# iyak/RNAelem

Hardware: AMD Instinct MI355X
Metric: train-iter seqs/sec (inside+outside) (higher is better)
Workload: dtype f64; 1 GPU; 10000 synthetic RNAs L=200, pattern ((.*.)), W=50 C=30 min_bpp=1e-4 T2004, x0 lambda=(1,1), one (fn,gr) eval per step; n_seq=10000, seq_len=200, pattern=((.*.)), bpp_filter=cached (computed once at load_batch, 0.1 s incl. plan), n_skipped=0

## Files before the change

rnaelem_amd/csrc/lin_kernels.hip:

```cpp
#include <hip/hip_runtime.h>

#include <algorithm>
#include <cstdio>
#include <cstdlib>
#include <type_traits>

#ifndef ELEMDP_KCI
#define ELEMDP_KCI 2
#endif
#ifndef ELEMDP_LB_IN
#define ELEMDP_LB_IN 4
#endif
#ifndef ELEMDP_LB_IN_FAST
#define ELEMDP_LB_IN_FAST 8
#endif
#ifndef ELEMDP_LB_CYK
#define ELEMDP_LB_CYK 8
#endif
#ifndef ELEMDP_LB_OUT6
#define ELEMDP_LB_OUT6 6
#endif
#ifndef ELEMDP_LB_OUT
#define ELEMDP_LB_OUT 4
#endif
#ifndef ELEMDP_BAND_THREADS
#define ELEMDP_BAND_THREADS 256
#endif
#ifndef ELEMDP_CPB_MAX
#define ELEMDP_CPB_MAX 64
#endif
#ifndef ELEMDP_KIB
#define ELEMDP_KIB 4
#endif
#ifndef ELEMDP_RECIN
#define ELEMDP_RECIN 1024
#endif
#ifndef ELEMDP_RECOUT
#define ELEMDP_RECOUT 960
#endif
#include "kernels.h"
#include "lin_rules.h"
#include "lin_fast.h"
#include "lin_views.h"
#include "scan_rules.h"
#include "wave_gather.h"

namespace elemdp {
namespace {
constexpr int kBT = ELEMDP_BAND_THREADS;
constexpr int kWaves = kBT / 64;

__device__ __forceinline__ int div_small(int q, int n) { return (int)(((float)q + 0.5f) * __frcp_rn((float)n)); }
__device__ __forceinline__ int div_rcp(int q, float rcp) { return (int)(((float)q + 0.5f) * rcp); }

__device__ __forceinline__ double rep_sum(const double* p, int nrep, int stride) {
  double a = p[0];
  for (int r = 1; r < nrep; ++r) a += p[r * stride];
  return a;
}

struct LinSink {
  double* en_;
  double eh0, eh1;
  int world = 0;
  double* pos0 = nullptr;
  double* pos1 = nullptr;
  double* pos2 = nullptr;
  __device__ __forceinline__ void en(int idx, double w) { atomicAdd(&en_[idx], w); }
  __device__ __forceinline__ void eh(int k, double w) { eh1 += k ? w : 0.; eh0 += k ? 0. : w; }
  __device__ __forceinline__ void pos(int which, int p, double w) {
    double* a = (which == 0) ? pos0 : (which == 1) ? pos1 : pos2;
    if (a) atomicAdd(&a[p], w);
  }
};

struct PhaseClock {
  long long* row;
  long long t0;
  __device__ __forceinline__ void start(long long* p) {
    row = p ? p + 16 * ((blockIdx.x + 7 * blockIdx.y) & 63) : nullptr;
    t0 = 0;
    if (row) t0 = __builtin_readcyclecounter();
  }
  template <int SLOT> __device__ __forceinline__ void mark() {
    if (row) {
      const long long t = __builtin_readcyclecounter();
      if (threadIdx.x == 0) atomicAdd((unsigned long long*)&row[SLOT], (unsigned long long)(t - t0));
      t0 = t;
    }
  }
  __device__ __forceinline__ void finish() {}
};

__device__ __forceinline__ void swizzled_block(unsigned& bx, unsigned& by) {
  const unsigned nbx = gridDim.x, total = gridDim.x * gridDim.y;
  const unsigned orig = blockIdx.y * nbx + blockIdx.x;
// ... 687 lines not shown
        const int xc = x < np ? x : np - 1;
        const LoopItem it = R.it[xc];
        const int meta = R.meta[xc];
        const int c = (meta >> 16) & 0x7fff;
        const int i = ci(c), j = i + d;
        const bool in_set = x < np && meta >= 0;
        const uint32_t rP = v.in.cidx(ST_P, it.l - it.k, it.k, 0), rL1 = v.in.cidx(ST_L, it.k - i, i, 0), rL2 = v.in.cidx(ST_L, j - it.l, it.l, 0);
        const double xw0 = R.xw[xc], xw1 = R.xw[R.cap + xc];
        double* hrow = heA + c * HD;
        const int qd = FAST ? A.fqd_in : A.qd_in;
        const int m0 = a.det ? __builtin_amdgcn_readfirstlane(G[qd + wv]) : 0;
        const int n_mine = a.det ? __builtin_amdgcn_readfirstlane(G[qd + wv + 1]) - m0 : (nq > wv ? (nq - wv + kWaves - 1) / kWaves : 0);
        for (int k0 = 0; k0 < n_mine; k0 += kTU) {
          int qa[kTU], qb[kTU];
          double x0[kTU], x1[kTU], x2[kTU];
#pragma unroll
          for (int u = 0; u < kTU; ++u) {
            const bool on = k0 + u < n_mine;
            const int kk = on ? k0 + u : 0;
            const int t = a.det ? __builtin_amdgcn_readfirstlane(G[qd + 5 + m0 + kk]) : wv + kWaves * kk;
            qa[u] = __builtin_amdgcn_readfirstlane(G[qc_in + 2 * t]);
            qb[u] = on ? __builtin_amdgcn_readfirstlane(G[qc_in + 2 * t + 1]) : (4 << 16);
            x0[u] = B[rP + (qa[u] & 0xff)]; x1[u] = B[rL1 + ((qa[u] >> 8) & 0xff)]; x2[u] = B[rL2 + ((qa[u] >> 16) & 0xff)];
          }
#pragma unroll
          for (int u = 0; u < kTU; ++u) {
            const double term = x0[u] * (x1[u] * x2[u]) * ((qb[u] & (1 << 16)) ? xw1 : xw0);
            if (!(qb[u] & (4 << 16)) && in_set && term != 0.) atomicAdd(&hrow[qb[u] & 0xffff], term);
          }
        }
      }
      __syncthreads();
    }
  }
  pc.mark<3>();
  const int NL = FAST ? A.n_lane : NA;
  if (tid < nc * NL && !(a.dbg & 4) && !(ELEMDP_KO & 4)) {
    const int c = div_rcp(tid, a.rcp_lane);
    const int s = FAST ? G[A.f_live_in + tid - c * NL] : tid - c * NL;
    const int i = ci(c);
    if (FAST) {
      fast_inside_unary<kFastR, FP, kFastL, CON, LPRE>(A, G + A.fp_in + s * kFastW, v.m.lin, v.in, crec + c * kCellInD, crfl[c], d, i, hb + c * HD + (tid - c * NL),
                                                 he + c * HD + (tid - c * NL), NW, 2 * CS, G + A.fs_in);
    } else {
      const Constraint con{CON ? a.ys[v.n] : -1, -1, 0};
      lin_inside_target_u<CON>(v.m, v.q, v.in, d, i, s, rep_sum(hb + c * HD + s, NW, 2 * CS), rep_sum(he + c * HD + s, NW, 2 * CS), con);
    }
  }
  pc.mark<4>();
  pc.finish();
}

constexpr int kLoopLanes = 64;
constexpr int kLoopColsMax = 16;
constexpr int kLoopProgW = 8;
static_assert(4 + kFastR <= kLoopProgW, "the staged program holds the right transitions");
static size_t loop_prepass_lds(const AutomatonLayout& A) {
  return sizeof(double) * (2 * (size_t)kLoopLanes * A.tab_rs[ST_L] + 5 * (size_t)A.n_wr) + sizeof(int32_t) * kLoopColsMax * kLoopProgW;
}
__global__ __launch_bounds__(kLoopLanes) void k4_in_loops(LinArgs a) {
  extern __shared__ double lds[];
  LViews v(a.lay);
  make_lviews(a, blockIdx.y, v);
  const AutomatonLayout& A = a.lay;
  const int tid = threadIdx.x, L = v.q.L, W = v.q.W;
  const int i0 = blockIdx.x * kLoopLanes;
  if (i0 > L) return;
  const int rs = v.in.rs[ST_L];
  double* cur = lds;
  double* prev = lds + kLoopLanes * rs;
  double* wr = lds + 2 * kLoopLanes * rs;
  int32_t* prog = reinterpret_cast<int32_t*>(wr + 5 * A.n_wr);
  for (int t = tid; t < kLoopColsMax * kLoopProgW; t += kLoopLanes) prog[t] = 0;
  for (int t = tid; t < 5 * A.n_wr; t += kLoopLanes) wr[t] = a.lin[A.lin_wr + t];
  __syncthreads();
  for (int k = tid; k < A.n_lane; k += kLoopLanes) {
    const int32_t* P = a.ints + A.fp_in + a.ints[A.f_live_in + k] * kFastW;
    const int c = fcol(P[2], 2);
    if (c >= 0 && c < kLoopColsMax)
      for (int w = 0; w < kLoopProgW; ++w) prog[c * kLoopProgW + w] = P[w];
  }
  __syncthreads();
  const int i = i0 + tid;
  const int dmax = (W < L - i0) ? W : L - i0;
  for (int d = 0; d <= dmax; ++d) {
    if (i + d <= L) {
      const int j = i + d;
      const int bj = d > 0 ? (int)v.q.seq[j - 1] : 0;
      const double ews_j = d > 0 ? v.q.ews[j - 1] : 1.;
      const int ub = v.q.ubits(i, d);
      for (int c = 0; c < rs; ++c)
        cur[tid * rs + c] = loop_inside_entry<kFastR>(prog + c * kLoopProgW, wr, prev + tid * rs, ub, d, bj, ews_j);
    }
    __syncthreads();
    const int nrows = (kLoopLanes < L - d - i0 + 1) ? kLoopLanes : L - d - i0 + 1;
    double* dst = v.in.band + v.in.cidx(ST_L, d, i0, 0);
    for (int t = tid; t < nrows * rs; t += kLoopLanes) dst[t] = cur[t];
    double* x = cur; cur = prev; prev = x;
  }
}

struct ExtLds { int lin, ews, blob, bits, seq8, unp8, total; };
__host__ __device__ inline ExtLds ext_lds(int nd, int n_lin, int Lmax, int nword, int n_stage) {
  ExtLds b;
  int o = nd * 8;
  b.lin = o; o += n_lin * 8;
  b.ews = o; o += (Lmax + 1) * 8;
  b.blob = o; o += n_stage * 4;
// ... 832 lines not shown
            op[u] = out.lda(d + 1, i, u < nr ? ce[u] & 0xff : p, u < nr);
          }
          double acc = 0.;
          if (a_in != 0.) {
            acc = tg != 0xff ? hp[c * HD + tg] : 0.;
            const double inz = a_in * (w1 ? pi.invZs : pi.invZ);
            const int bj = step ? (int)v.q.seq[j] : 0;
            const double ewj = step ? v.q.ews[j] : 1.;
            double* en = l_en + (w1 ? nt : 0);
#pragma unroll
            for (int u = 0; u < kFastR; ++u)
              if (u < nr) {
                const int id = (ce[u] >> 8) & 0x7fff;
                const double term = op[u] * (v.m.lin[A.lin_wr + 5 * id + bj] * ((G[A.fe_r + 2 * id + 1] & 1) ? ewj : 1.));
                const double z = term * inz;
                if ((MODE == OUT_SCAN || MODE == OUT_END) &&
                    !fast_scan_stat<MODE, false, true>(sink, G[A.fs_out + id], i - 1, j, false, MODE == OUT_END && j == a.ys[v.n], L == j + 1, z))
                  continue;
                if (MODE != OUT_END && !v.m.no_prf && z != 0. && bj) atomicAdd(&en[G[A.fe_r + 2 * id] + bj], z);
                acc += term;
              }
          }
          out.a(d, i, p) = acc;
        }
        continue;
      }
      const int tgt = v.m.ints[A.ap_tgt + p];
      const bool w1 = pi.merged && v.m.ints[A.ap_t + p] == A.shadow;
      sink.en_ = l_en + (w1 ? nt : 0);
      LinOutCtx<LinSink> x{v.m, v.q, in, out, w1 ? pi.invZs : pi.invZ, sink, Constraint{MODE == OUT_END ? a.ys[v.n] : -1, -1, 0}};
      lin_outside_apair<MODE>(x, d, i0 + c, p, tgt >= 0 ? hp[c * HD + tgt] : 0.);
    }
    sink.en_ = en_keep;
  }
  pc.mark<11>();
  if (MODE == OUT_SCAN || MODE == OUT_END) {
    __syncthreads();
    const int p1 = (i0 + nc + d < L) ? i0 + nc + d : L;
    for (int t = tid; t <= p1 - pos_p0; t += kBT) {
      const double v0 = l_pos[t], v1 = l_pos[win + t];
      if (MODE == OUT_SCAN) {
        if (v0 != 0. && pos_p0 + t < L) atomicAdd(&a.pos_start[v.seq_base + pos_p0 + t], v0);
        if (v1 != 0. && pos_p0 + t < L) atomicAdd(&a.pos_inner[v.seq_base + pos_p0 + t], v1);
      } else if (v0 != 0.) {
        atomicAdd(&a.pos_end[v.pos_base + pos_p0 + t], v0);
      }
    }
  }
  if (MODE == OUT_TRAIN || MODE == OUT_SCAN) lflush(a, v, pi, sink, l_en0, kBT, (int)bx);
  pc.mark<12>();
  pc.finish();
}

constexpr int kRowsT = 8, kRowsMax = 32, kSeedCap = 256, kSeedBatch = 2;
static_assert(2 * kRowsMax <= 64, "the runs of a tile are scanned by one wave");
__host__ __device__ inline int loop_rows_r(int rs) { const int r = kBT / (rs > 0 ? rs : 1); return r < kRowsMax ? r : kRowsMax; }
static size_t loop_rows_lds(const AutomatonLayout& A) {
  const size_t rs = A.tab_rs[ST_L], R = loop_rows_r(A.tab_rs[ST_L]);
  return sizeof(double) * (R * (kRowsT + 1) * rs + 2 * kSeedCap + (R + kRowsT) + 5 * (size_t)A.n_wr + 2 * (size_t)A.n_theta + 4) +
         sizeof(int32_t) * (2 * R * (kRowsT + 1) + 2 * R + 1 + 4 * kSeedCap + 4 * (size_t)A.n_quad + (size_t)A.n_lane + kLoopColsMax * (kLoopProgW + 1) + (R + kRowsT));
}
__global__ __launch_bounds__(kBT) void k4_out_lrows(LinArgs a) {
  extern __shared__ double lds[];
  unsigned bx, by;
  swizzled_block(bx, by);
  LViews v(a.lay);
  make_lviews(a, by, v);
  const LPass pi = lpass(a, v);
  if (pi.skip) return;
  const AutomatonLayout& A = a.lay;
  const int tid = threadIdx.x, L = v.q.L, W = v.q.W, nt = A.n_theta, nq = A.n_quad, HD = A.n_lane;
  const int rs = v.out.rs[ST_L], R = loop_rows_r(rs), TS = (kRowsT + 1) * rs;
  const int i0 = bx * R;
  if (i0 > L) return;
  const int nrow = (R < L - i0 + 1) ? R : L - i0 + 1, nrr = 2 * nrow;
  double* acc = lds;
  double* s_xw = acc + R * TS;
  double* s_ew = s_xw + 2 * kSeedCap;
  double* wr = s_ew + R + kRowsT;
  double* l_en = wr + 5 * A.n_wr;
  int* offs = reinterpret_cast<int*>(l_en + 2 * nt + 4);
  int* pre = offs + 2 * R * (kRowsT + 1);
  int* s_row = pre + 2 * R + 1;
  int* tq = s_row + 4 * kSeedCap;
  int* lcol = tq + 4 * nq;
  int32_t* prog = lcol + HD;
  int32_t* pst = prog + kLoopColsMax * kLoopProgW;
  int* s_b = pst + kLoopColsMax;
  const int32_t* G = v.m.big;
  for (int t = tid; t < kLoopColsMax * (kLoopProgW + 1); t += kBT) prog[t] = 0;
  for (int t = tid; t < 5 * A.n_wr; t += kBT) wr[t] = a.lin[A.lin_wr + t];
  for (int t = tid; t < 2 * nt + 4; t += kBT) l_en[t] = 0.;
  for (int t = tid; t < 4 * nq; t += kBT) tq[t] = G[A.fqc_out + 2 * nq + t];
  __syncthreads();
  for (int k = tid; k < HD; k += kBT) {
    const int s = a.ints[A.f_live_out + k];
    const int32_t* P = a.ints + A.fp_out + s * kFastW;
    const int c = fcol(P[2], 2);
    lcol[k] = (c >= 0 && c < rs) ? c : -1;
    if (c >= 0 && c < kLoopColsMax) {
      for (int w = 0; w < kLoopProgW; ++w) prog[c * kLoopProgW + w] = P[w];
      pst[c] = s;
    }
  }
  __syncthreads();
  const int r = tid / rs, c = tid - r * rs, i = i0 + r;
  const bool lane = r < R;
  const int32_t* P = prog + (lane ? c : 0) * kLoopProgW;
  const int w0 = P[0];
  const bool have = lane && i <= L && (w0 & 1);
  const bool w1 = pi.merged && pst[lane ? c : 0] == A.shadow;
  const int kl = (w0 >> 2) & 1, cEo = fcol(P[1], 1), ehs = v.m.lam_same ? 0 : kl;
  const double invZ = w1 ? pi.invZs : pi.invZ;
  int enr[kFastR], fr[kFastR];
#pragma unroll
  for (int u = 0; u < kFastR; ++u) {
    const bool on = u < ((w0 >> 8) & 15);
    const int id = on ? (P[4 + u] >> 16) & 0x7fff : 0;
    enr[u] = on ? G[A.fe_r + 2 * id] : 0;
    fr[u] = on ? G[A.fe_r + 2 * id + 1] : 0;
  }
  LinSink sink;
  sink.world = w1 ? 1 : 0;
  sink.en_ = l_en + (w1 ? nt : 0);
  sink.eh0 = sink.eh1 = 0.;
  double* const row_e = acc + (lane ? r * TS + c : 0);
  const float rcp_nq = 1.0f / (float)(nq > 0 ? nq : 1);
  const double* IB = v.in.band;
  const double* OB = v.out.band;
  const int dmax = (W < L - i0) ? W : L - i0;
  double carry = 0.;
  for (int dhi = dmax; dhi >= 0; dhi -= kRowsT) {
    const int d0 = dhi >= kRowsT ? dhi - kRowsT + 1 : 0, nd = dhi - d0 + 1;
    double inL[kRowsT], t6[kRowsT];
    {
      int ub[kRowsT];
      uint32_t pw[kRowsT];
#pragma unroll
      for (int dd = 0; dd < kRowsT; ++dd) {
        const int d = d0 + dd;
        const bool in = have && dd < nd && i + d <= L;
        const bool up = in && i > 0 && d + 2 <= W && i + d + 1 <= L;
        ub[dd] = v.q.ubits(in ? i : 0, in ? d : 0);
        ub[dd] = in ? ub[dd] : 0;
        pw[dd] = v.q.okbits[up ? (uint32_t)v.q.cell(i - 1, d + 2) >> 5 : 0u];
        pw[dd] = up ? pw[dd] : 0u;
      }
#pragma unroll
      for (int dd = 0; dd < kRowsT; ++dd) {
        const int d = d0 + dd, c_up = v.q.cell(i - 1, d + 2);
        const bool on = (ub[dd] & UB_L) != 0, eok = on && ((pw[dd] >> (c_up & 31)) & 1u);
        inL[dd] = v.in.ldc(ST_L, d, i, c, on);
        const double oE = v.out.ldc(ST_E, d, i, cEo, eok), xhp = xw_cell(v.q, kl, XT_HP, eok ? c_up : 0), ehp = v.q.e_hp[eok ? c_up : 0];
        t6[dd] = 0.;
        if (eok && inL[dd] != 0.) t6[dd] = loop_outside_cell(inL[dd], oE, xhp, ehp, invZ, ehs, sink);
      }
    }
    if (lane) {
#pragma unroll
      for (int dd = 0; dd < kRowsT; ++dd) row_e[dd * rs] = dd == nd ? carry : t6[dd];
      row_e[kRowsT * rs] = carry;
    }
    {
      constexpr int kOffU = (2 * kRowsMax * (kRowsT + 1) + kBT - 1) / kBT;
      int ov[kOffU], os[kOffU];
#pragma unroll
      for (int u = 0; u < kOffU; ++u) {
        const int t = tid + u * kBT;
        const bool ok = t < nrr * (nd + 1) && nq > 0;
        const int rr = ok ? div_small(t, nd + 1) : 0, dd = ok ? t - rr * (nd + 1) : 0, role = rr >= nrow, d = d0 + dd;
        const int32_t* off = role ? v.q.by_right_off : v.q.by_left_off;
        os[u] = t < nrr * (nd + 1) ? rr * (kRowsT + 1) + dd : -1;
        ov[u] = off[ok ? v.q.cell(i0 + rr - role * nrow, d > 0 ? d : 1) : 0];
        ov[u] = ok ? ov[u] : 0;
      }
      int lo = 0, hi = 0;
      if (tid < 64) {
        const bool ok = tid < nrr && nq > 0;
        const int role = tid >= nrow, ri = i0 + tid - role * nrow;
        const int32_t* off = role ? v.q.by_right_off : v.q.by_left_off;
        lo = off[ok ? v.q.cell(ri, d0 > 0 ? d0 : 1) : 0];
        hi = off[ok ? v.q.cell(ri, d0 + nd) : 0];
        lo = ok ? lo : 0;
        hi = ok ? hi : 0;
      }
      int jb = 0;
      double jw = 0.;
      if (tid < nrow + nd) {
        const int j = i0 + d0 + tid;
        jb = j < L ? (int)v.q.seq[j] : 0;
        jw = v.q.ews[j < L ? j : L];
      }
#pragma unroll
      for (int u = 0; u < kOffU; ++u)
        if (os[u] >= 0) offs[os[u]] = ov[u];
      if (tid < 64) {
        int n = hi - lo;
#pragma unroll
        for (int sft = 1; sft < 64; sft <<= 1) {
          const int up = __shfl_up(n, sft);
          if (tid >= sft) n += up;
        }
        if (tid < nrr) pre[tid + 1] = n;
        if (tid == 0) pre[0] = 0;
      }
      if (tid < nrow + nd) { s_b[tid] = jb; s_ew[tid] = jw; }
    }
    __syncthreads();
    const int n_rec = pre[nrr];
    for (int p0 = 0; p0 < n_rec; p0 += kSeedCap) {
      const int np = (kSeedCap < n_rec - p0) ? kSeedCap : n_rec - p0;
      for (int xs = tid; xs < np; xs += kBT) {
        const int x = p0 + xs;
        int rr = 0;
        while (rr + 1 < nrr && pre[rr + 1] <= x) ++rr;
        const int* ro = offs + rr * (kRowsT + 1);
        const int n = ro[0] + (x - pre[rr]);
        int dd = 0;
        while (dd + 1 < nd && ro[dd + 1] <= n) ++dd;
        const int role = rr >= nrow, rw = rr - role * nrow, ri = i0 + rw, d = d0 + dd;
        const bool on = ri + d <= L && (v.q.ubits(ri, d) & UB_L);
        const LoopItem it = (role ? v.q.items_right : v.q.items_left)[n];
        s_row[xs] = (int)v.out.cidx(ST_E, it.j - it.i, it.i, 0);
        s_row[kSeedCap + xs] = (int)v.in.cidx(ST_P, it.l - it.k, it.k, 0);
        s_row[2 * kSeedCap + xs] = (int)(role ? v.in.cidx(ST_L, it.k - it.i, it.i, 0) : v.in.cidx(ST_L, it.j - it.l, it.l, 0));
        s_row[3 * kSeedCap + xs] = on ? 2 * (rw * TS + dd * rs) + role : -1;
        s_xw[xs] = lin_weight(v.m.lambda[0], it.tsc);
        s_xw[kSeedCap + xs] = lin_weight(v.m.lambda[1], it.tsc);
      }
      __syncthreads();
      for (int wb = tid; wb < np * nq; wb += kSeedBatch * kBT) {
        double x0[kSeedBatch], x1[kSeedBatch], x2[kSeedBatch], xw[kSeedBatch];
        int dst[kSeedBatch];
#pragma unroll
        for (int u = 0; u < kSeedBatch; ++u) {
          const int w = wb + u * kBT;
          const bool in = w < np * nq;
          const int xs = in ? div_rcp(w, rcp_nq) : 0, t = in ? w - xs * nq : 0;
          const int cell = s_row[3 * kSeedCap + xs];
          const int32_t* q2 = tq + (cell & 1) * 2 * nq + 2 * t;
          const int qa = q2[0], qb = q2[1], col = lcol[qb & 0xffff];
          const bool ok = in && cell >= 0 && col >= 0 && !(qb & (4 << 16));
          dst[u] = ok ? (cell >> 1) + col : -1;
          x0[u] = OB[ok ? (uint32_t)s_row[xs] + (qa & 0xff) : 0u];
          x1[u] = IB[ok ? (uint32_t)s_row[kSeedCap + xs] + ((qa >> 8) & 0xff) : 0u];
          x2[u] = IB[ok ? (uint32_t)s_row[2 * kSeedCap + xs] + ((qa >> 16) & 0xff) : 0u];
          xw[u] = s_xw[((qb >> 16) & 1) * kSeedCap + xs];
        }
#pragma unroll
        for (int u = 0; u < kSeedBatch; ++u)
          if (dst[u] >= 0) {
            const double term = loop_outside_seed_term(x0[u], x1[u], x2[u], xw[u]);
            if (term != 0.) atomicAdd(&acc[dst[u]], term);
          }
      }
      __syncthreads();
    }
    double oL = carry;
#pragma unroll
    for (int dd = kRowsT - 1; dd >= 0; --dd) {
      if (dd >= nd) continue;
      oL = 0.;
      if (inL[dd] != 0.) {
        const int d = d0 + dd, j = i + d;
        double sL = 0.;
        if (j < L && d + 1 <= W)
          sL = loop_outside_chain<kFastR>(P, enr, fr, wr, row_e + (dd + 1) * rs - c, inL[dd], s_b[r + dd], s_ew[r + dd], invZ, v.m.no_prf != 0, sink);
        oL = row_e[dd * rs] + sL;
      }
      if (lane) row_e[dd * rs] = oL;
      __syncthreads();
    }
    carry = oL;
  }
  lflush(a, v, pi, sink, l_en, kBT, (int)bx);
}

__global__ __launch_bounds__(kThreads) void k4_combine(LinArgs a, int G) {
  const int g = blockIdx.x;
  if (g >= G) return;
  const int n = a.grp[g];
  double* row = a.seq_out + (size_t)n * a.out_stride;
  if (row[4] != 0.) return;
  const double* zs = a.zs + (size_t)g * 4;
  const int nt = a.lay.n_theta;
  if (a.det) {
    const double* dr = a.det_rows + (size_t)n * a.det_nslot * a.out_stride;
    for (int t = 6 + threadIdx.x; t < 6 + 2 * nt + 4; t += kThreads) {
      double acc = 0.;
      for (int k = 0; k < a.det_nslot; ++k) acc += dr[(size_t)k * a.out_stride + t];
      row[t] = acc;
    }
    __syncthreads();
  }
  const bool positive = a.plans[n].positive != 0;
  const double pa = zs[1] / zs[0], pn = zs[2] / zs[0];
  for (int t = threadIdx.x; t < nt + 2; t += kThreads) {
    double* A = (t < nt) ? &row[6 + t] : &row[6 + 2 * nt + (t - nt)];
    double* B = (t < nt) ? &row[6 + nt + t] : &row[6 + 2 * nt + 2 + (t - nt)];
    const double va = *A, vb = *B;
    if (a.schedule == 1) {
      const double full = pa * va + pn * vb;
      if (a.lik_ratio && !positive) { *A = va; *B = full; }
      else { *A = full; *B = positive ? va : vb; }
    } else if (a.lik_ratio && !positive) {
      *A = vb; *B = va;
    }
  }
}

__device__ __forceinline__ unsigned long long cyk_key(double v) {
  const long long b = __double_as_longlong(v + 0.);
  return (unsigned long long)(b >= 0 ? b : (b ^ 0x7fffffffffffffffLL)) ^ 0x8000000000000000ULL;
}
__device__ __forceinline__ double cyk_unkey(unsigned long long k) {
  const long long b = (long long)(k ^ 0x8000000000000000ULL);
  return __longlong_as_double(b >= 0 ? b : (b ^ 0x7fffffffffffffffLL));
}

__global__ __launch_bounds__(kThreads) void k5_cyk_serial(LinArgs a) {
  __shared__ AutomatonLayout s_lay;
  stage_layout(a, &s_lay, kThreads);
  unsigned bx, by;
  swizzled_block(bx, by);
  LViews v(s_lay);
  make_lviews(a, by, v);
// ... 340 lines not shown
  switch (k4_form(a, lds, 6, fast, big)) {
    case K4_FP2_WAVES: hipLaunchKernelGGL((k4_out<MODE, true, true, 2, true>), grid, dim3(kBT), lds, st, a); break;
    case K4_FP2: hipLaunchKernelGGL((k4_out<MODE, true, true, 2>), grid, dim3(kBT), lds, st, a); break;
    case K4_FAST: hipLaunchKernelGGL((k4_out<MODE, true, true>), grid, dim3(kBT), lds, st, a); break;
    case K4_STAGED: hipLaunchKernelGGL((k4_out<MODE, true>), grid, dim3(kBT), lds, st, a); break;
    case K4_GENERIC: hipLaunchKernelGGL((k4_out<MODE, false>), grid, dim3(kBT), lds, st, a); break;
  }
}
template <>
void launch_k4_out<OUT_NONE>(const LinArgs& a, dim3 grid, size_t lds, bool, bool, hipStream_t st) {
  hipLaunchKernelGGL((k4_out<OUT_NONE, true>), grid, dim3(kBT), lds, st, a);
}

struct GroupGeom {
  LinArgs a;
  bool big, fast;
  int hd, win;
  size_t lds_in, lds_out;
  bool stage_ext;
  size_t lds_ext_in;
  int ext_nt;
};
static bool geometry_fast(const LinArgs& a) {
  return a.fast && a.n_stage >= a.lay.n_ints && a.lay.fp_ok && !(a.dbg & 16) && a.lay.lin_total <= 2048;
}
int lin_train_cpb(const LinArgs& full) {
  return geometry_fast(full) ? std::min(kBT / std::max(full.lay.n_lane, 1), ELEMDP_CPB_MAX) : 0;
}
int lin_live_span_max() { return kLiveSpanMax; }
bool lin_loop_prepass_ok(const AutomatonLayout& A, const int32_t* ints, int min_span) {
  const bool say = getenv("ELEMDP_PLAN_DEBUG") != nullptr;
  if (!A.fp_ok || A.tab_rs[ST_L] < 1 || A.tab_rs[ST_L] > kLoopColsMax || loop_prepass_lds(A) > 64 * 1024) {
    if (say) fprintf(stderr, "loop pre-pass: not for this automaton (fp_ok %d, L row of %d columns)\n", A.fp_ok, A.tab_rs[ST_L]);
    return false;
  }
  auto col = [](int packed, int byte) { const int c = (packed >> (8 * byte)) & 0xff; return c == 0xff ? -1 : c; };
  unsigned seen = 0;
  for (int k = 0; k < A.n_lane; ++k) {
    const int32_t* P = ints + A.fp_in + ints[A.f_live_in + k] * kFastW;
    const int c = col(P[2], 2);
    if (c >= 0) {
      if (c >= A.tab_rs[ST_L] || ((seen >> c) & 1u)) { if (say) fprintf(stderr, "loop pre-pass: not for this automaton (column %d of lane %d)\n", c, k); return false; }
      seen |= 1u << c;
      continue;
    }
    if (!(P[0] & 1) || col(P[1], 1) < 0) continue;
    const int nR = (P[0] >> 8) & 15;
    bool zero = !(P[0] & 2) || min_span > 2;
    for (int u = 0; u < nR && u < kFastR; ++u) zero = zero && col(P[4 + u], 0) < 0;
    if (!zero) { if (say) fprintf(stderr, "loop pre-pass: not for this automaton (lane %d: a loop state with an E column, no L column and an L value)\n", k); return false; }
  }
  return true;
}
static bool loop_outside_lds_ok(const AutomatonLayout& A) {
  return A.tab_rs[ST_L] >= 1 && A.tab_rs[ST_L] <= kLoopColsMax && A.tab_rs[ST_L] <= kBT && loop_rows_lds(A) <= 64 * 1024;
}
bool lin_loop_outside_ok(const AutomatonLayout& A, const int32_t* ints) {
  const bool say = getenv("ELEMDP_PLAN_DEBUG") != nullptr;
  if (!A.fp_ok || !loop_outside_lds_ok(A)) {
    if (say) fprintf(stderr, "L kernel behind the outside sweep: not for this automaton (fp_ok %d, L row of %d columns, LDS %zu)\n", A.fp_ok, A.tab_rs[ST_L], loop_rows_lds(A));
    return false;
  }
  auto col = [](int packed, int byte) { const int c = (packed >> (8 * byte)) & 0xff; return c == 0xff ? -1 : c; };
  unsigned seen = 0;
  for (int k = 0; k < A.n_lane; ++k) {
    const int s = ints[A.f_live_out + k];
    const int c = col(ints[A.fp_out + s * kFastW + 2], 2), ci = col(ints[A.fp_in + s * kFastW + 2], 2);
    if (c != ci || (c >= 0 && (c >= A.tab_rs[ST_L] || ((seen >> c) & 1u)))) {
      if (say) fprintf(stderr, "L kernels behind the outside sweep: not for this automaton (state %d: L column %d outside, %d inside)\n", s, c, ci);
      return false;
    }
    if (c >= 0) seen |= 1u << c;
  }
  return true;
}
static GroupGeom group_geometry(const LinArgs& full, int G, int Lmax, int Wmax, bool scan) {
  GroupGeom g;
  LinArgs& a = g.a;
  a = full;
  const int S = a.lay.S, nt = a.lay.n_theta;
  a.cpb = std::min(kBT / S, ELEMDP_CPB_MAX);
  a.wmax = Wmax;
  a.ext_ring = G <= 1024 ? 1 : 0;
  a.lmax = Lmax;
  if (scan) { a.schedule = 0; a.pass = 0; a.scan = 1; a.det = 0; }
  g.big = a.n_stage >= a.lay.n_ints;
  const bool fast = g.fast = geometry_fast(a);
  a.fast = fast ? 1 : 0;
  if (fast) a.cpb = std::min(kBT / std::max(a.lay.n_lane, 1), ELEMDP_CPB_MAX);
  a.n_lin = fast ? a.lay.lin_total : kLinEth + nt;
  const int NW = a.det ? kBT / 64 : 1;
  g.hd = fast ? a.lay.n_lane : S;
  set_rcps(a, fast);
  if (scan || !fast || a.det || !a.p.useful || !a.p.blocks || !a.blk_grid || a.live_span < a.cpb) { a.p.blocks = nullptr; a.blk_grid = nullptr; a.live_span = 0; }
  if (scan || !fast || !a.p.useful) a.loop_pre = 0;
  if (a.loop_pre && a.p.blocks && (!a.p.blocks_in || !a.blk_grid_in)) a.loop_pre = 0;
  if (scan || !fast || !a.p.useful || a.det) a.loop_post = 0;
  if (a.loop_post && a.p.blocks && (!a.p.blocks_in || !a.blk_grid_in)) a.loop_post = 0;
  if (a.loop_post && !loop_outside_lds_ok(a.lay)) a.loop_post = 0;
  const int sp = a.live_span > a.cpb ? a.live_span : a.cpb;
  g.win = sp + Wmax + 3;
  g.lds_in = block_lds(2 * a.cpb * g.hd + kRecIn, a.cpb, a.n_lin, g.win, fast ? a.lay.fb_in_n : staged_ints(a.lay, a.n_stage, 0), 0, fast ? kCellInD : 0, sp).total;
  g.lds_out = block_lds(out_doubles(a.cpb * g.hd, nt, g.win, NW, scan), a.cpb, a.n_lin, g.win, fast ? a.lay.fb_out_n : staged_ints(a.lay, a.n_stage, 1), 3 * a.cpb, fast ? kCellOutD : 0, sp).total;
  g.stage_ext = Lmax <= 2048 && a.nword_max <= 8192;
  g.lds_ext_in = g.stage_ext ? (size_t)ext_lds((a.ext_ring ? ext_ring_doubles(0, Wmax, S, kLinEth + nt, Lmax, a.nword_max, a.n_stage) : 0), kLinEth + nt, Lmax, a.nword_max, a.n_stage).total : 0;
  g.ext_nt = (a.ext_block == kExtBlock && a.ext_ring && a.lay.n_active <= 128 && !(a.dbg & 8192)) ? 128 * kExtBlock : 128;
  return g;
}
static unsigned band_blocks(LinArgs& a, int ncell, bool train) {
  const int n = (ncell + a.cpb - 1) / a.cpb;
  if (!train || !a.blk_grid || !a.p.blocks) return (unsigned)n;
  if (a.blk_grid[a.d] < 0) { a.p.blocks = nullptr; return (unsigned)n; }
  if (a.zeros_kept && a.blk_grid[a.d] == 0) return 0u;
  return (unsigned)std::max(1, std::min(n, a.blk_grid[a.d]));
}
template <bool CON>
static void inside_sweeps(GroupGeom& g, int G, int Lmax, int Wmax, bool bands, hipStream_t st) {
  LinArgs& a = g.a;
  const bool pre = !CON && bands && g.fast && a.loop_pre;
  LinArgs ai = a;
  if (!pre) ai.loop_pre = 0;
  if (pre) {
    if (a.p.blocks) { ai.p.blocks = a.p.blocks_in; ai.blk_grid = a.blk_grid_in; }
    hipLaunchKernelGGL(k4_in_loops, dim3((Lmax + kLoopLanes) / kLoopLanes, G), dim3(kLoopLanes), loop_prepass_lds(a.lay), st, ai);
  }
  if (bands)
    for (int d = pre ? a.in_d0 : 0; d <= Wmax; ++d) {
      const int ncell = Lmax - d + 1;
      if (ncell <= 0) break;
      LinArgs ad = ai;
      ad.d = d;
      const unsigned gx = band_blocks(ad, ncell, !CON);
      if (!gx) continue;
      launch_k4_in<CON>(ad, dim3(gx, G), g.lds_in, g.fast, g.big, st);
    }
  if (g.stage_ext) hipLaunchKernelGGL((k4_in_ext<true, CON>), dim3(G), dim3(g.ext_nt), g.lds_ext_in, st, a);
  else hipLaunchKernelGGL((k4_in_ext<false, CON>), dim3(G), dim3(128), 0, st, a);
}
template <int MODE>
static void outside_bands(GroupGeom& g, int G, int Lmax, int Wmax, hipStream_t st) {
  LinArgs& a = g.a;
  hipLaunchKernelGGL(k4_r7, dim3(((Lmax + 1) * (Wmax + 1) + kThreads - 1) / kThreads, G), dim3(kThreads), 0, st, a);
  const bool post = MODE == OUT_TRAIN && g.fast && a.loop_post;
  LinArgs ao = a;
  if (!post) ao.loop_post = 0;
  if (post && a.p.blocks) { ao.p.blocks = a.p.blocks_in; ao.blk_grid = a.blk_grid_in; }
  for (int d = Wmax; d >= (post ? a.in_d0 : 0); --d) {
    const int ncell = Lmax - d + 1;
    if (ncell <= 0) continue;
    LinArgs ad = ao;
    ad.d = d;
    const unsigned gx = band_blocks(ad, ncell, MODE == OUT_TRAIN);
    if (!gx) continue;
    launch_k4_out<MODE>(ad, dim3(gx, G), g.lds_out, g.fast, g.big, st);
  }
  if (post) {
    const int rows = loop_rows_r(a.lay.tab_rs[ST_L]);
    hipLaunchKernelGGL(k4_out_lrows, dim3((Lmax + rows) / rows, G), dim3(kBT), loop_rows_lds(a.lay), st, a);
  }
}
template <int MODE>
static void scan_outside(GroupGeom& g, int G, int Lmax, int Wmax, hipStream_t st) {
  const LinArgs& a = g.a;
  const int S = a.lay.S, nt = a.lay.n_theta;
  const size_t lds_ext_out = g.stage_ext ? (size_t)ext_lds(2 * nt + 4 + (a.ext_ring ? ext_ring_doubles(2 * nt + 4, Wmax, S, kLinEth + nt, Lmax, a.nword_max, a.n_stage) : 0), kLinEth + nt, Lmax, a.nword_max, a.n_stage).total : sizeof(double) * (2 * nt + 4);
  if (g.stage_ext) hipLaunchKernelGGL((k4_out_ext<MODE, true>), dim3(G), dim3(g.ext_nt), lds_ext_out, st, a);
  else hipLaunchKernelGGL((k4_out_ext<MODE, false>), dim3(G), dim3(128), lds_ext_out, st, a);
  outside_bands<MODE>(g, G, Lmax, Wmax, st);
}
template <bool CON, int MODE>
static void scan_sweeps(GroupGeom& g, int G, int Lmax, int Wmax, hipStream_t st) {
  inside_sweeps<CON>(g, G, Lmax, Wmax, true, st);
  scan_outside<MODE>(g, G, Lmax, Wmax, st);
}

hipError_t launch_lin_scan_group(const LinArgs& full, int G, int Lmax, int Wmax, ScanPass pass, hipStream_t st) {
  if (G <= 0) return hipSuccess;
  GroupGeom g = group_geometry(full, G, Lmax, Wmax, true);
  const LinArgs& a = g.a;
  if (getenv("ELEMDP_LDS_DEBUG") && pass == SCAN_PASS_START) fprintf(stderr, "scan group: G %d cpb %d S %d nt %d fast %d n_lin %d fast blob in/out %d/%d ints win %d lds k4_in %zu k4_out %zu\n", G, a.cpb, a.lay.S, a.lay.n_theta, (int)g.fast, a.n_lin, a.lay.fb_in_n, a.lay.fb_out_n, g.win, g.lds_in, g.lds_out);
  if (pass == SCAN_PASS_INSIDE) {
    inside_sweeps<false>(g, G, Lmax, Wmax, true, st);
  } else if (pass == SCAN_PASS_START) {
    scan_sweeps<false, OUT_SCAN>(g, G, Lmax, Wmax, st);
    hipLaunchKernelGGL(k5_pick<0>, dim3((G + 63) / 64), dim3(64), 0, st, a, G);
  } else if (pass == SCAN_PASS_OUT_ARI || pass == SCAN_PASS_OUT_NASI) {
    g.a.scan_terms = pass == SCAN_PASS_OUT_ARI ? 1 : 2;
    scan_outside<OUT_SCAN>(g, G, Lmax, Wmax, st);
  } else {
    scan_sweeps<true, OUT_END>(g, G, Lmax, Wmax, st);
    hipLaunchKernelGGL(k5_pick<1>, dim3((G + 63) / 64), dim3(64), 0, st, a, G);
  }
  return hipGetLastError();
}

hipError_t launch_lin_group(const LinArgs& full, int G, int Lmax, int Wmax, bool first_pass_only, hipStream_t st) {
  if (G <= 0) return hipSuccess;
  GroupGeom g = group_geometry(full, G, Lmax, Wmax, false);
  const LinArgs& a = g.a;
  const int S = a.lay.S, nt = a.lay.n_theta;
  inside_sweeps<false>(g, G, Lmax, Wmax, !a.no_rss, st);
  const int n_pass = (a.schedule == 1 || first_pass_only) ? 1 : 2;
  const bool combine = (a.schedule == 1 || a.lik_ratio || a.det) && !first_pass_only;
  if (getenv("ELEMDP_LDS_DEBUG")) {
    const bool stats = !(g.big && (a.dbg & 16));
    fprintf(stderr, "lin group: G %d cpb %d fast %d n_lin %d staged ints in/out %d/%d lds k4_in %zu k4_out %zu fp_max_p %d forms k4_in %s k4_out %s stage_ext %d ext_nt %d ext_ring %d n_pass %d combine %d\n", G, a.cpb, (int)g.fast, a.n_lin, staged_ints(a.lay, a.n_stage, 0), staged_ints(a.lay, a.n_stage, 1), g.lds_in, g.lds_out, a.lay.fp_max_p,
            a.no_rss ? "none" : kK4FormName[k4_form(a, g.lds_in, 8, g.fast, g.big)], a.no_rss ? "none" : !stats ? "nostat" : kK4FormName[k4_form(a, g.lds_out, 6, g.fast, g.big)],
            (int)g.stage_ext, g.stage_ext ? g.ext_nt : 128, a.ext_ring, n_pass, (int)combine);
    fprintf(stderr, "lin group: loop_prepass %d loop_outside %d (k4_out_lrows lds %zu, %d rows x %d diagonals)\n", a.loop_pre, a.loop_post, loop_rows_lds(a.lay), loop_rows_r(a.lay.tab_rs[ST_L]), kRowsT);
  }
  for (int pass = 0; pass < n_pass; ++pass) {
    GroupGeom gp = g;
    LinArgs& b = gp.a;
    b.pass = pass;
    const int n_stat = ext_stat_doubles(nt, b.det);
    if (g.stage_ext) hipLaunchKernelGGL((k4_out_ext<OUT_TRAIN, true>), dim3(G), dim3(b.det ? 128 : g.ext_nt), (size_t)ext_lds(n_stat + (b.ext_ring ? ext_ring_doubles(n_stat, Wmax, S, kLinEth + nt, Lmax, b.nword_max, b.n_stage) : 0), kLinEth + nt, Lmax, b.nword_max, b.n_stage).total, st, b);
    else hipLaunchKernelGGL((k4_out_ext<OUT_TRAIN, false>), dim3(G), dim3(128), sizeof(double) * n_stat, st, b);
    if (b.no_rss) continue;
    if (g.big && (b.dbg & 16)) outside_bands<OUT_NONE>(gp, G, Lmax, Wmax, st);
    else outside_bands<OUT_TRAIN>(gp, G, Lmax, Wmax, st);
  }
  if (combine) hipLaunchKernelGGL(k4_combine, dim3(G), dim3(kThreads), 0, st, a, G);
  return hipGetLastError();
}

}
```

Baseline: 52930 seq/s.

## Stage loop-row metadata in LDS once per block in k4_out_lrows

The loop-row outside kernel now loads the unpaired bits, ok-bit words, sequence bases, edge weights and per-tile record offsets and prefix sums into shared memory once, before the diagonal-tile loop. Previously it recomputed them with global loads and an extra barrier on every tile. The per-record row search becomes a binary search over the staged prefix sums, and the per-diagonal offset table is dropped by deriving d from the loop item itself. In exchange, LDS now grows with W through a new layout header, which may lower occupancy or rule out the kernel for large windows. Phase-clock marks are also added.

```diff
diff --git a/rnaelem_amd/csrc/lin_kernels.hip b/rnaelem_amd/csrc/lin_kernels.hip
--- a/rnaelem_amd/csrc/lin_kernels.hip
+++ b/rnaelem_amd/csrc/lin_kernels.hip
@@ -42,6 +42,7 @@
 #include "lin_rules.h"
 #include "lin_fast.h"
 #include "lin_views.h"
+#include "loop_rows_layout.h"
 #include "scan_rules.h"
 #include "wave_gather.h"
 
@@ -835,8 +836,6 @@
 }
 
 constexpr int kLoopLanes = 64;
-constexpr int kLoopColsMax = 16;
-constexpr int kLoopProgW = 8;
 static_assert(4 + kFastR <= kLoopProgW, "the staged program holds the right transitions");
 static size_t loop_prepass_lds(const AutomatonLayout& A) {
   return sizeof(double) * (2 * (size_t)kLoopLanes * A.tab_rs[ST_L] + 5 * (size_t)A.n_wr) + sizeof(int32_t) * kLoopColsMax * kLoopProgW;
@@ -1775,13 +1774,10 @@
   pc.finish();
 }
 
-constexpr int kRowsT = 8, kRowsMax = 32, kSeedCap = 256, kSeedBatch = 2;
 static_assert(2 * kRowsMax <= 64, "the runs of a tile are scanned by one wave");
-__host__ __device__ inline int loop_rows_r(int rs) { const int r = kBT / (rs > 0 ? rs : 1); return r < kRowsMax ? r : kRowsMax; }
-static size_t loop_rows_lds(const AutomatonLayout& A) {
-  const size_t rs = A.tab_rs[ST_L], R = loop_rows_r(A.tab_rs[ST_L]);
-  return sizeof(double) * (R * (kRowsT + 1) * rs + 2 * kSeedCap + (R + kRowsT) + 5 * (size_t)A.n_wr + 2 * (size_t)A.n_theta + 4) +
-         sizeof(int32_t) * (2 * R * (kRowsT + 1) + 2 * R + 1 + 4 * kSeedCap + 4 * (size_t)A.n_quad + (size_t)A.n_lane + kLoopColsMax * (kLoopProgW + 1) + (R + kRowsT));
+static_assert(kBT == kLoopRowsThreads && kSeedCap <= kBT, "the layout's workgroup; a record per lane");
+static size_t loop_rows_lds(const AutomatonLayout& A, int W) {
+  return (size_t)loop_rows_lds_bytes(A.tab_rs[ST_L], W, A.n_wr, A.n_theta, A.n_quad, A.n_lane);
 }
 __global__ __launch_bounds__(kBT) void k4_out_lrows(LinArgs a) {
   extern __shared__ double lds[];
@@ -1791,30 +1787,71 @@
   make_lviews(a, by, v);
   const LPass pi = lpass(a, v);
   if (pi.skip) return;
+  PhaseClock pc;
+  pc.start(a.prof);
   const AutomatonLayout& A = a.lay;
   const int tid = threadIdx.x, L = v.q.L, W = v.q.W, nt = A.n_theta, nq = A.n_quad, HD = A.n_lane;
   const int rs = v.out.rs[ST_L], R = loop_rows_r(rs), TS = (kRowsT + 1) * rs;
   const int i0 = bx * R;
   if (i0 > L) return;
   const int nrow = (R < L - i0 + 1) ? R : L - i0 + 1, nrr = 2 * nrow;
-  double* acc = lds;
-  double* s_xw = acc + R * TS;
-  double* s_ew = s_xw + 2 * kSeedCap;
-  double* wr = s_ew + R + kRowsT;
-  double* l_en = wr + 5 * A.n_wr;
-  int* offs = reinterpret_cast<int*>(l_en + 2 * nt + 4);
-  int* pre = offs + 2 * R * (kRowsT + 1);
-  int* s_row = pre + 2 * R + 1;
-  int* tq = s_row + 4 * kSeedCap;
-  int* lcol = tq + 4 * nq;
-  int32_t* prog = lcol + HD;
-  int32_t* pst = prog + kLoopColsMax * kLoopProgW;
-  int* s_b = pst + kLoopColsMax;
+  const LoopRowsLds y = loop_rows_layout(rs, a.wmax, A.n_wr, nt, nq, HD);
+  char* const lds8 = reinterpret_cast<char*>(lds);
+  double* acc = reinterpret_cast<double*>(lds8 + y.acc.off);
+  double* s_xw = reinterpret_cast<double*>(lds8 + y.xw.off);
+  double* s_ew = reinterpret_cast<double*>(lds8 + y.ew.off);
+  double* wr = reinterpret_cast<double*>(lds8 + y.wr.off);
+  double* l_en = reinterpret_cast<double*>(lds8 + y.en.off);
+  int* s_lo = reinterpret_cast<int*>(lds8 + y.lo.off);
+  int* s_pre = reinterpret_cast<int*>(lds8 + y.pre.off);
+  int* s_row = reinterpret_cast<int*>(lds8 + y.srow.off);
+  int* tq = reinterpret_cast<int*>(lds8 + y.tq.off);
+  int* lcol = reinterpret_cast<int*>(lds8 + y.lcol.off);
+  int32_t* prog = reinterpret_cast<int32_t*>(lds8 + y.prog.off);
+  int32_t* pst = reinterpret_cast<int32_t*>(lds8 + y.pst.off);
+  uint32_t* s_okw = reinterpret_cast<uint32_t*>(lds8 + y.okw.off);
+  uint8_t* s_pb = reinterpret_cast<uint8_t*>(lds8 + y.pb.off);
+  uint8_t* s_ub = reinterpret_cast<uint8_t*>(lds8 + y.ub.off);
   const int32_t* G = v.m.big;
+  const int dmax = (W < L - i0) ? W : L - i0;
+  const int okw0 = (i0 > 0 ? (i0 - 1) * (W + 1) : 0) >> 5;
   for (int t = tid; t < kLoopColsMax * (kLoopProgW + 1); t += kBT) prog[t] = 0;
   for (int t = tid; t < 5 * A.n_wr; t += kBT) wr[t] = a.lin[A.lin_wr + t];
   for (int t = tid; t < 2 * nt + 4; t += kBT) l_en[t] = 0.;
   for (int t = tid; t < 4 * nq; t += kBT) tq[t] = G[A.fqc_out + 2 * nq + t];
+  for (int t = tid; t < (dmax + 1) * R; t += kBT) {
+    const int d = div_small(t, R), rw = t - d * R;
+    const bool in = i0 + rw + d <= L;
+    const int ub = v.q.ubits(in ? i0 + rw : 0, in ? d : 0);
+    s_ub[t] = (uint8_t)(in ? ub : 0);
+  }
+  {
+    const int last_bit = (i0 + R - 2) * (W + 1) + W, end_bit = (L + 1) * (W + 1) - 1;
+    const int okw1 = (last_bit < end_bit ? (last_bit > 0 ? last_bit : 0) : end_bit) >> 5;
+    for (int t = tid; t <= okw1 - okw0 && t < y.nokw; t += kBT) s_okw[t] = v.q.okbits[okw0 + t];
+  }
+  for (int t = tid; t < R + dmax; t += kBT) {
+    const int j = i0 + t;
+    s_pb[t] = j < L ? v.q.seq[j] : (uint8_t)0;
+    s_ew[t] = v.q.ews[j < L ? j : L];
+  }
+  for (int tt = tid >> 6; tt <= dmax / kRowsT; tt += kWaves) {
+    const int ln = tid & 63, dhi = dmax - tt * kRowsT, d0 = dhi >= kRowsT ? dhi - kRowsT + 1 : 0;
+    const bool ok = ln < nrr && nq > 0;
+    const int role = ln >= nrow, ri = i0 + ln - role * nrow;
+    const int32_t* off = role ? v.q.by_right_off : v.q.by_left_off;
+    int lo = off[ok ? v.q.cell(ri, d0 > 0 ? d0 : 1) : 0], hi = off[ok ? v.q.cell(ri, dhi + 1) : 0];
+    lo = ok ? lo : 0;
+    hi = ok ? hi : 0;
+    int n = hi - lo;
+#pragma unroll
+    for (int sft = 1; sft < 64; sft <<= 1) {
+      const int up = __shfl_up(n, sft);
+      if (ln >= sft) n += up;
+    }
+    if (ln < nrr) { s_lo[tt * 2 * R + ln] = lo; s_pre[tt * (2 * R + 1) + ln + 1] = n; }
+    if (ln == 0) s_pre[tt * (2 * R + 1)] = 0;
+  }
   __syncthreads();
   for (int k = tid; k < HD; k += kBT) {
     const int s = a.ints[A.f_live_out + k];
@@ -1851,99 +1888,47 @@
   const float rcp_nq = 1.0f / (float)(nq > 0 ? nq : 1);
   const double* IB = v.in.band;
   const double* OB = v.out.band;
-  const int dmax = (W < L - i0) ? W : L - i0;
   double carry = 0.;
-  for (int dhi = dmax; dhi >= 0; dhi -= kRowsT) {
+  pc.mark<7>();
+  for (int dhi = dmax, tt = 0; dhi >= 0; dhi -= kRowsT, ++tt) {
     const int d0 = dhi >= kRowsT ? dhi - kRowsT + 1 : 0, nd = dhi - d0 + 1;
+    const int* const pre = s_pre + tt * (2 * R + 1);
+    const int* const rlo = s_lo + tt * 2 * R;
     double inL[kRowsT], t6[kRowsT];
-    {
-      int ub[kRowsT];
-      uint32_t pw[kRowsT];
-#pragma unroll
-      for (int dd = 0; dd < kRowsT; ++dd) {
-        const int d = d0 + dd;
-        const bool in = have && dd < nd && i + d <= L;
-        const bool up = in && i > 0 && d + 2 <= W && i + d + 1 <= L;
-        ub[dd] = v.q.ubits(in ? i : 0, in ? d : 0);
-        ub[dd] = in ? ub[dd] : 0;
-        pw[dd] = v.q.okbits[up ? (uint32_t)v.q.cell(i - 1, d + 2) >> 5 : 0u];
-        pw[dd] = up ? pw[dd] : 0u;
-      }
-#pragma unroll
-      for (int dd = 0; dd < kRowsT; ++dd) {
-        const int d = d0 + dd, c_up = v.q.cell(i - 1, d + 2);
-        const bool on = (ub[dd] & UB_L) != 0, eok = on && ((pw[dd] >> (c_up & 31)) & 1u);
-        inL[dd] = v.in.ldc(ST_L, d, i, c, on);
-        const double oE = v.out.ldc(ST_E, d, i, cEo, eok), xhp = xw_cell(v.q, kl, XT_HP, eok ? c_up : 0), ehp = v.q.e_hp[eok ? c_up : 0];
-        t6[dd] = 0.;
-        if (eok && inL[dd] != 0.) t6[dd] = loop_outside_cell(inL[dd], oE, xhp, ehp, invZ, ehs, sink);
-      }
+#pragma unroll
+    for (int dd = 0; dd < kRowsT; ++dd) {
+      const int d = d0 + dd, c_up = v.q.cell(i - 1, d + 2);
+      const bool in = have && dd < nd && i + d <= L;
+      const bool up = in && i > 0 && d + 2 <= W && i + d + 1 <= L;
+      const bool on = (s_ub[in ? d * R + r : 0] & UB_L) != 0 && in;
+      const bool eok = on && up && ((s_okw[up ? (c_up >> 5) - okw0 : 0] >> (c_up & 31)) & 1u);
+      inL[dd] = v.in.ldc(ST_L, d, i, c, on);
+      const double oE = v.out.ldc(ST_E, d, i, cEo, eok), xhp = xw_cell(v.q, kl, XT_HP, eok ? c_up : 0), ehp = v.q.e_hp[eok ? c_up : 0];
+      t6[dd] = 0.;
+      if (eok && inL[dd] != 0.) t6[dd] = loop_outside_cell(inL[dd], oE, xhp, ehp, invZ, ehs, sink);
     }
     if (lane) {
 #pragma unroll
       for (int dd = 0; dd < kRowsT; ++dd) row_e[dd * rs] = dd == nd ? carry : t6[dd];
       row_e[kRowsT * rs] = carry;
     }
-    {
-      constexpr int kOffU = (2 * kRowsMax * (kRowsT + 1) + kBT - 1) / kBT;
-      int ov[kOffU], os[kOffU];
-#pragma unroll
-      for (int u = 0; u < kOffU; ++u) {
-        const int t = tid + u * kBT;
-        const bool ok = t < nrr * (nd + 1) && nq > 0;
-        const int rr = ok ? div_small(t, nd + 1) : 0, dd = ok ? t - rr * (nd + 1) : 0, role = rr >= nrow, d = d0 + dd;
-        const int32_t* off = role ? v.q.by_right_off : v.q.by_left_off;
-        os[u] = t < nrr * (nd + 1) ? rr * (kRowsT + 1) + dd : -1;
-        ov[u] = off[ok ? v.q.cell(i0 + rr - role * nrow, d > 0 ? d : 1) : 0];
-        ov[u] = ok ? ov[u] : 0;
-      }
-      int lo = 0, hi = 0;
-      if (tid < 64) {
-        const bool ok = tid < nrr && nq > 0;
-        const int role = tid >= nrow, ri = i0 + tid - role * nrow;
-        const int32_t* off = role ? v.q.by_right_off : v.q.by_left_off;
-        lo = off[ok ? v.q.cell(ri, d0 > 0 ? d0 : 1) : 0];
-        hi = off[ok ? v.q.cell(ri, d0 + nd) : 0];
-        lo = ok ? lo : 0;
-        hi = ok ? hi : 0;
-      }
-      int jb = 0;
-      double jw = 0.;
-      if (tid < nrow + nd) {
-        const int j = i0 + d0 + tid;
-        jb = j < L ? (int)v.q.seq[j] : 0;
-        jw = v.q.ews[j < L ? j : L];
-      }
-#pragma unroll
-      for (int u = 0; u < kOffU; ++u)
-        if (os[u] >= 0) offs[os[u]] = ov[u];
-      if (tid < 64) {
-        int n = hi - lo;
-#pragma unroll
-        for (int sft = 1; sft < 64; sft <<= 1) {
-          const int up = __shfl_up(n, sft);
-          if (tid >= sft) n += up;
-        }
-        if (tid < nrr) pre[tid + 1] = n;
-        if (tid == 0) pre[0] = 0;
-      }
-      if (tid < nrow + nd) { s_b[tid] = jb; s_ew[tid] = jw; }
-    }
-    __syncthreads();
+    pc.mark<2>();
     const int n_rec = pre[nrr];
+    if (n_rec == 0) __syncthreads();
     for (int p0 = 0; p0 < n_rec; p0 += kSeedCap) {
       const int np = (kSeedCap < n_rec - p0) ? kSeedCap : n_rec - p0;
       for (int xs = tid; xs < np; xs += kBT) {
         const int x = p0 + xs;
-        int rr = 0;
-        while (rr + 1 < nrr && pre[rr + 1] <= x) ++rr;
-        const int* ro = offs + rr * (kRowsT + 1);
-        const int n = ro[0] + (x - pre[rr]);
-        int dd = 0;
-        while (dd + 1 < nd && ro[dd + 1] <= n) ++dd;
-        const int role = rr >= nrow, rw = rr - role * nrow, ri = i0 + rw, d = d0 + dd;
-        const bool on = ri + d <= L && (v.q.ubits(ri, d) & UB_L);
+        int rr = 0, rhi = nrr - 1;
+        while (rr < rhi) {
+          const int mid = (rr + rhi + 1) >> 1;
+          if (pre[mid] <= x) rr = mid; else rhi = mid - 1;
+        }
+        const int n = rlo[rr] + (x - pre[rr]);
+        const int role = rr >= nrow, rw = rr - role * nrow;
         const LoopItem it = (role ? v.q.items_right : v.q.items_left)[n];
+        const int d = role ? it.j - it.l : it.k - it.i, dd = d - d0;
+        const bool on = dd >= 0 && dd < nd && (s_ub[dd >= 0 && dd < nd ? d * R + rw : 0] & UB_L);
         s_row[xs] = (int)v.out.cidx(ST_E, it.j - it.i, it.i, 0);
         s_row[kSeedCap + xs] = (int)v.in.cidx(ST_P, it.l - it.k, it.k, 0);
         s_row[2 * kSeedCap + xs] = (int)(role ? v.in.cidx(ST_L, it.k - it.i, it.i, 0) : v.in.cidx(ST_L, it.j - it.l, it.l, 0));
@@ -1952,6 +1937,7 @@
         s_xw[kSeedCap + xs] = lin_weight(v.m.lambda[1], it.tsc);
       }
       __syncthreads();
+      pc.mark<13>();
       for (int wb = tid; wb < np * nq; wb += kSeedBatch * kBT) {
         double x0[kSeedBatch], x1[kSeedBatch], x2[kSeedBatch], xw[kSeedBatch];
         int dst[kSeedBatch];
@@ -1978,6 +1964,7 @@
           }
       }
       __syncthreads();
+      pc.mark<14>();
     }
     double oL = carry;
 #pragma unroll
@@ -1988,13 +1975,14 @@
         const int d = d0 + dd, j = i + d;
         double sL = 0.;
         if (j < L && d + 1 <= W)
-          sL = loop_outside_chain<kFastR>(P, enr, fr, wr, row_e + (dd + 1) * rs - c, inL[dd], s_b[r + dd], s_ew[r + dd], invZ, v.m.no_prf != 0, sink);
+          sL = loop_outside_chain<kFastR>(P, enr, fr, wr, row_e + (dd + 1) * rs - c, inL[dd], (int)s_pb[r + d], s_ew[r + d], invZ, v.m.no_prf != 0, sink);
         oL = row_e[dd * rs] + sL;
       }
       if (lane) row_e[dd * rs] = oL;
       __syncthreads();
     }
     carry = oL;
+    pc.mark<15>();
   }
   lflush(a, v, pi, sink, l_en, kBT, (int)bx);
 }
@@ -2441,13 +2429,13 @@
   }
   return true;
 }
-static bool loop_outside_lds_ok(const AutomatonLayout& A) {
-  return A.tab_rs[ST_L] >= 1 && A.tab_rs[ST_L] <= kLoopColsMax && A.tab_rs[ST_L] <= kBT && loop_rows_lds(A) <= 64 * 1024;
+static bool loop_outside_lds_ok(const AutomatonLayout& A, int W) {
+  return loop_rows_fits(A.tab_rs[ST_L], W, A.n_wr, A.n_theta, A.n_quad, A.n_lane);
 }
 bool lin_loop_outside_ok(const AutomatonLayout& A, const int32_t* ints) {
   const bool say = getenv("ELEMDP_PLAN_DEBUG") != nullptr;
-  if (!A.fp_ok || !loop_outside_lds_ok(A)) {
-    if (say) fprintf(stderr, "L kernel behind the outside sweep: not for this automaton (fp_ok %d, L row of %d columns, LDS %zu)\n", A.fp_ok, A.tab_rs[ST_L], loop_rows_lds(A));
+  if (!A.fp_ok || !loop_outside_lds_ok(A, 0)) {
+    if (say) fprintf(stderr, "L kernel behind the outside sweep: not for this automaton (fp_ok %d, L row of %d columns, LDS %zu)\n", A.fp_ok, A.tab_rs[ST_L], loop_rows_lds(A, 0));
     return false;
   }
   auto col = [](int packed, int byte) { const int c = (packed >> (8 * byte)) & 0xff; return c == 0xff ? -1 : c; };
@@ -2486,7 +2474,7 @@
   if (a.loop_pre && a.p.blocks && (!a.p.blocks_in || !a.blk_grid_in)) a.loop_pre = 0;
   if (scan || !fast || !a.p.useful || a.det) a.loop_post = 0;
   if (a.loop_post && a.p.blocks && (!a.p.blocks_in || !a.blk_grid_in)) a.loop_post = 0;
-  if (a.loop_post && !loop_outside_lds_ok(a.lay)) a.loop_post = 0;
+  if (a.loop_post && !loop_outside_lds_ok(a.lay, Wmax)) a.loop_post = 0;
   const int sp = a.live_span > a.cpb ? a.live_span : a.cpb;
   g.win = sp + Wmax + 3;
   g.lds_in = block_lds(2 * a.cpb * g.hd + kRecIn, a.cpb, a.n_lin, g.win, fast ? a.lay.fb_in_n : staged_ints(a.lay, a.n_stage, 0), 0, fast ? kCellInD : 0, sp).total;
@@ -2545,7 +2533,7 @@
   }
   if (post) {
     const int rows = loop_rows_r(a.lay.tab_rs[ST_L]);
-    hipLaunchKernelGGL(k4_out_lrows, dim3((Lmax + rows) / rows, G), dim3(kBT), loop_rows_lds(a.lay), st, a);
+    hipLaunchKernelGGL(k4_out_lrows, dim3((Lmax + rows) / rows, G), dim3(kBT), loop_rows_lds(a.lay, a.wmax), st, a);
   }
 }
 template <int MODE>
@@ -2596,7 +2584,7 @@
     fprintf(stderr, "lin group: G %d cpb %d fast %d n_lin %d staged ints in/out %d/%d lds k4_in %zu k4_out %zu fp_max_p %d forms k4_in %s k4_out %s stage_ext %d ext_nt %d ext_ring %d n_pass %d combine %d\n", G, a.cpb, (int)g.fast, a.n_lin, staged_ints(a.lay, a.n_stage, 0), staged_ints(a.lay, a.n_stage, 1), g.lds_in, g.lds_out, a.lay.fp_max_p,
             a.no_rss ? "none" : kK4FormName[k4_form(a, g.lds_in, 8, g.fast, g.big)], a.no_rss ? "none" : !stats ? "nostat" : kK4FormName[k4_form(a, g.lds_out, 6, g.fast, g.big)],
             (int)g.stage_ext, g.stage_ext ? g.ext_nt : 128, a.ext_ring, n_pass, (int)combine);
-    fprintf(stderr, "lin group: loop_prepass %d loop_outside %d (k4_out_lrows lds %zu, %d rows x %d diagonals)\n", a.loop_pre, a.loop_post, loop_rows_lds(a.lay), loop_rows_r(a.lay.tab_rs[ST_L]), kRowsT);
+    fprintf(stderr, "lin group: loop_prepass %d loop_outside %d (k4_out_lrows lds %zu, %d rows x %d diagonals)\n", a.loop_pre, a.loop_post, loop_rows_lds(a.lay, a.wmax), loop_rows_r(a.lay.tab_rs[ST_L]), kRowsT);
   }
   for (int pass = 0; pass < n_pass; ++pass) {
     GroupGeom gp = g;
diff --git a/rnaelem_amd/csrc/loop_rows_layout.h b/rnaelem_amd/csrc/loop_rows_layout.h
--- /dev/null
+++ b/rnaelem_amd/csrc/loop_rows_layout.h
@@ -0,0 +1,81 @@
+#pragma once
+
+#if defined(__HIPCC__)
+#define ELEMDP_LRL __host__ __device__ inline
+#else
+#define ELEMDP_LRL inline
+#endif
+
+namespace elemdp {
+
+constexpr int kLoopRowsThreads = 256;
+constexpr int kLoopColsMax = 16;
+constexpr int kLoopProgW = 8;
+constexpr int kRowsT = 8, kRowsMax = 32, kSeedCap = 256, kSeedBatch = 2;
+constexpr int kLoopRowsLdsMax = 64 * 1024;
+
+ELEMDP_LRL int loop_rows_r(int rs) { const int r = kLoopRowsThreads / (rs > 0 ? rs : 1); return r < kRowsMax ? r : kRowsMax; }
+
+struct LdsRegion { int off, bytes, align; };
+struct LoopRowsLds {
+  int rows, tiles, npos, nokw;
+  LdsRegion acc;
+  LdsRegion xw;
+  LdsRegion ew;
+  LdsRegion wr;
+  LdsRegion en;
+  LdsRegion lo;
+  LdsRegion pre;
+  LdsRegion srow;
+  LdsRegion tq;
+  LdsRegion lcol;
+  LdsRegion prog;
+  LdsRegion pst;
+  LdsRegion okw;
+  LdsRegion pb;
+  LdsRegion ub;
+  int total;
+};
+constexpr int kLoopRowsRegions = 15;
+
+ELEMDP_LRL LoopRowsLds loop_rows_layout(int rs, int W, int n_wr, int n_theta, int n_quad, int n_lane) {
+  LoopRowsLds y;
+  const int R = loop_rows_r(rs);
+  y.rows = R;
+  y.tiles = W / kRowsT + 1;
+  y.npos = R + W;
+  y.nokw = (R * (W + 1) + 31) / 32 + 1;
+  int o = 0;
+  auto take = [&o](LdsRegion& g, int bytes, int align) {
+    o = (o + align - 1) / align * align;
+    g.off = o; g.bytes = bytes; g.align = align;
+    o += bytes;
+  };
+  take(y.acc, 8 * R * (kRowsT + 1) * rs, 8);
+  take(y.xw, 8 * 2 * kSeedCap, 8);
+  take(y.ew, 8 * y.npos, 8);
+  take(y.wr, 8 * 5 * n_wr, 8);
+  take(y.en, 8 * (2 * n_theta + 4), 8);
+  take(y.lo, 4 * y.tiles * 2 * R, 4);
+  take(y.pre, 4 * y.tiles * (2 * R + 1), 4);
+  take(y.srow, 4 * 4 * kSeedCap, 4);
+  take(y.tq, 4 * 4 * n_quad, 4);
+  take(y.lcol, 4 * n_lane, 4);
+  take(y.prog, 4 * kLoopColsMax * kLoopProgW, 4);
+  take(y.pst, 4 * kLoopColsMax, 4);
+  take(y.okw, 4 * y.nokw, 4);
+  take(y.pb, y.npos, 1);
+  take(y.ub, R * (W + 1), 1);
+  y.total = (o + 7) / 8 * 8;
+  return y;
+}
+inline void loop_rows_regions(const LoopRowsLds& y, LdsRegion out[kLoopRowsRegions]) {
+  const LdsRegion all[kLoopRowsRegions] = {y.acc, y.xw, y.ew, y.wr, y.en, y.lo, y.pre, y.srow, y.tq, y.lcol, y.prog, y.pst, y.okw, y.pb, y.ub};
+  for (int k = 0; k < kLoopRowsRegions; ++k) out[k] = all[k];
+}
+ELEMDP_LRL int loop_rows_lds_bytes(int rs, int W, int n_wr, int n_theta, int n_quad, int n_lane) { return loop_rows_layout(rs, W, n_wr, n_theta, n_quad, n_lane).total; }
+ELEMDP_LRL bool loop_rows_fits(int rs, int W, int n_wr, int n_theta, int n_quad, int n_lane) {
+  return rs >= 1 && rs <= kLoopColsMax && rs <= kLoopRowsThreads && W >= 0 && loop_rows_lds_bytes(rs, W, n_wr, n_theta, n_quad, n_lane) <= kLoopRowsLdsMax;
+}
+
+}
```

Measured after the change: 54320 seq/s, median of 6. +2.6%, better.
